# andreaskoepf/CLIP-Image-Captioning

Measured on NVIDIA B200. Metric: captions/sec (GPT2-XL, prefix 40, 32 tok), higher is better.
Workload: dtype bf16

## Files before the change

### clip-image-captioning_b200/csrc/engine.cu

```cuda
#include <stdarg.h>
#include <stdio.h>
#include <stdlib.h>
#include <string.h>

#include <algorithm>

#include "engine.h"

using namespace ccb;

namespace {

thread_local char g_create_err[512] = "";

int fail(ccb_ctx* c, const char* fmt, ...) {
  char buf[512];
  va_list ap;
  va_start(ap, fmt);
  vsnprintf(buf, sizeof(buf), fmt, ap);
  va_end(ap);
  if (c)
    c->err = buf;
  else
    snprintf(g_create_err, sizeof(g_create_err), "%s", buf);
// ... 397 lines not shown
  p.tbl_entries = m.tbl_entries;
  for (int k = 0; k < 4; ++k) p.g[k] = m.g[k];
  p.h = c->h;
  p.x = c->x;
  p.att = c->att;
  p.mlp = c->mlp;
  p.ws = m.d_ws;
  p.wte = c->wte;
  p.wpe = c->wpe;
  p.tokens = c->next_tokens;
  p.ctx_len = c->ctx_len;
  p.block_table = c->block_table;
  p.kv = c->kv;
  p.lnf_g = c->lm_lnf.g;
  p.lnf_b = c->lm_lnf.b;
  p.sync = m.d_sync;
  p.sc_cap = (c->max_pages_per_row + 3) & ~3;
  p.trace = m.trace;
  p.log2_page_tokens = 0;
  while ((1 << p.log2_page_tokens) < c->kv.page_tokens) ++p.log2_page_tokens;
  RUN(mega_launch(p, s));
  return 0;
}

int lm_decode_step(ccb_ctx* c, int rows, cudaStream_t s) {
  const ccb_model_desc& D = c->desc;
  const int d = D.lm_d, H = D.lm_heads, hd = d / H;
  if (c->mega.available && rows <= c->mega.max_rows && c->mega.enabled && (c->kv.page_tokens & (c->kv.page_tokens - 1)) == 0) {
    if (lm_decode_layers_mega(c, rows, s)) return -1;
    RUN(linear(c, c->x, d, rows, c->lm_head, CCB_ACT_NONE, nullptr, 0, c->logits, c->ldv, 0, s));
    return 0;
  }
  RUN(embed_tokens(c->wte, D.lm_arch == CCB_LM_GPT2 ? c->wpe : nullptr, c->next_tokens, c->ctx_len, c->h, rows, d, D.lm_vocab, D.lm_n_pos, s));
  const BlockShape sh = lm_shape(D);
  const float scale = 1.0f / sqrtf(static_cast<float>(hd));
  static const bool fuse_out = [] {
    const char* e = getenv("CCB_GPTJ_FUSE_OUT");
    return !(e && e[0] == '0');
  }();
  for (int l = 0; l < D.lm_layers; ++l) {
    const Block& b = c->lm[l];
    if (sh.parallel && fuse_out && b.projfc2.w != nullptr && c->attmlp != nullptr) {
      const long long ldc = 5LL * d;
      RUN(layernorm_f32_bf16(c->h, d, b.ln1.g, b.ln1.b, sh.eps, c->x, d, rows, d, s));
      RUN(linear(c, c->x, d, rows, b.qkv, CCB_ACT_NONE, nullptr, 0, c->qkv, 3 * d, 1, s));
      RUN(attention_decode(c->qkv, c->attmlp, ldc, rows, H, hd, scale, &c->kv, l, c->block_table, c->ctx_len, D.lm_rotary_dim, s));
      RUN(linear(c, c->x, d, rows, b.fc, sh.act, nullptr, 0, c->attmlp + d, ldc, 1, s));
      RUN(linear(c, c->attmlp, ldc, rows, b.projfc2, CCB_ACT_NONE, c->h, d, c->h, d, 0, s));
      continue;
    }
    auto attn = [&]() {
      return attention_decode(c->qkv, c->att, d, rows, H, hd, scale, &c->kv, l, c->block_table, c->ctx_len,
                              D.lm_rotary_dim, s);
    };
    if (block_forward(c, b, rows, sh, attn, s)) return -1;
  }
  RUN(layernorm_f32_bf16(c->h, d, c->lm_lnf.g, c->lm_lnf.b, D.lm_ln_eps, c->x, d, rows, d, s));
  RUN(linear(c, c->x, d, rows, c->lm_head, CCB_ACT_NONE, nullptr, 0, c->logits, c->ldv, 0, s));
  return 0;
}

SampleParams sample_params(ccb_ctx* c, const ccb_gen_params* p, int rows) {
  SampleParams sp;
  sp.temperature = p->temperature;
  sp.top_p = p->top_p;
  sp.top_k = p->top_k;
  sp.top_p_rows = p->top_p_rows;
  sp.top_k_rows = p->top_k_rows;
  sp.typ_p = p->typ_p;
  sp.typ_p_rows = p->typ_p_rows;
  sp.repetition_penalty = p->repetition_penalty;
  sp.q_noise = p->q_noise;
  sp.ldq = p->q_ld;
  sp.q_step_stride = static_cast<long long>(rows) * p->q_ld;
  sp.seed = p->seed;
  sp.row_ids = reinterpret_cast<const long long*>(p->row_ids);
  (void)c;
  return sp;
}

int select_step(ccb_ctx* c, const ccb_gen_params* p, int rows, int T, bool after_prefill, cudaStream_t s) {
  const int V = c->desc.lm_vocab;
  if (p->mode == CCB_GEN_GREEDY) {
    RUN(sample_greedy(c->logits, c->ldv, rows, V, c->next_tokens, s));
  } else {
    SampleParams sp = sample_params(c, p, rows);
    sp.history = c->gen_tokens;
    sp.ld_hist = T;
    sp.hist_len_from_step = 1;
    sp.step = c->step;
    RUN(sample_top_p(c->logits, c->ldv, rows, V, sp, c->next_tokens, s));
  }
  RUN(advance_rows(c->next_tokens, rows, c->gen_tokens, T, c->lengths, c->stops, c->finished,
                   after_prefill ? nullptr : c->ctx_len, c->step, p->stop_token, p->max_stops, p->eos_token, s));
  return 0;
}

int beam_select(ccb_ctx* c, const ccb_gen_params* p, int N, int T, bool first, cudaStream_t s) {
  const int beam = p->beam_size, rows = N * beam;
  if (!first) RUN(increment_rows(c->ctx_len, rows, c->step, s));
  BeamState st;
  st.scores = c->scores;
  st.seq_lengths = c->seq_lengths;
  st.has_stopped = c->has_stopped;
  st.tokens = c->gen_tokens;
  st.max_len = T;
  st.step = c->step;
  st.cand_scratch = c->beam_cand;
  st.cand_rows = c->max_rows;
  if (c->capturing) c->capture_launches++; else c->launches++;
  RUN(beam_step(c->logits, c->ldv, N, beam, c->desc.lm_vocab, p->temperature, p->stop_token, st, c->next_tokens,
                c->src_rows, c->block_table, c->max_pages_per_row, c->ctx_len, s));
  return 0;
}

int decode_iteration(ccb_ctx* c, const ccb_gen_params* p, int N, int rows, int T, cudaStream_t s) {
  if (lm_decode_step(c, rows, s)) return -1;
  if (p->mode == CCB_GEN_BEAM) return beam_select(c, p, N, T, false, s);
  return select_step(c, p, rows, T, false, s);
}

std::string graph_key(const ccb_gen_params* p, int N, int rows, int T, int c_mega) {
  char buf[512];
  snprintf(buf, sizeof(buf), "g%d m%d N%d r%d T%d st%d ms%d eos%d t%a p%a k%d rp%a b%d seed%llu q%p ld%lld ids%p pr%p kr%p ty%a tr%p",
           c_mega, p->mode, N, rows, T, p->stop_token, p->max_stops, p->eos_token, p->temperature, p->top_p, p->top_k,
           p->repetition_penalty, p->beam_size, static_cast<unsigned long long>(p->seed),
           static_cast<const void*>(p->q_noise), static_cast<long long>(p->q_ld), static_cast<const void*>(p->row_ids),
           static_cast<const void*>(p->top_p_rows), static_cast<const void*>(p->top_k_rows), p->typ_p,
           static_cast<const void*>(p->typ_p_rows));
  return buf;
}

int generate_on_work_stream(ccb_ctx* c, const ccb_gen_params* p, const float* embeds, int N, int S0,
                            int32_t* tokens_out, int32_t* lengths_out, float* scores_out) {
  const ccb_model_desc& D = c->desc;
  cudaStream_t s = c->work;
  const bool is_beam = p->mode == CCB_GEN_BEAM;
  const int beam = is_beam ? p->beam_size : 1;
  const int rows = N * beam;
  const int T = p->max_new_tokens;
  if (p->mode != CCB_GEN_GREEDY && p->mode != CCB_GEN_SAMPLE && !is_beam) return fail(c, "generate: unknown mode %d", p->mode);
  if (N <= 0 || N > D.max_images) return fail(c, "generate: N=%d outside [1, max_images=%d]", N, D.max_images);
  if (beam < 1 || beam > D.max_beam || beam > 8) return fail(c, "generate: beam_size=%d outside [1, max_beam=%d]", beam, D.max_beam);
  if (T <= 0 || S0 <= 0 || S0 + T > D.max_ctx) return fail(c, "generate: S0=%d + max_new_tokens=%d exceeds max_ctx=%d", S0, T, D.max_ctx);
  if (N * S0 > D.max_lm_tokens) return fail(c, "generate: N*S0=%d exceeds max_lm_tokens=%d", N * S0, D.max_lm_tokens);
  if (const char* why = attention_prefill_unsupported(S0, D.lm_d / D.lm_heads, 1, true, D.lm_rotary_dim, false))
    return fail(c, "generate: prefix of S0=%d tokens with head_dim %d: %s", S0, D.lm_d / D.lm_heads, why);

  const int page_tokens = is_beam ? 1 : D.page_tokens;
  const int pages_per_row = is_beam ? (S0 + T) : (S0 + T + page_tokens - 1) / page_tokens;
  const long long need_tokens = is_beam ? static_cast<long long>(N) * (S0 + static_cast<long long>(beam) * T)
                                        : static_cast<long long>(rows) * pages_per_row * page_tokens;
  if (need_tokens > c->kv_pool_tokens) return fail(c, "generate: KV pool too small (%lld > %lld tokens)", need_tokens, c->kv_pool_tokens);
  c->kv.page_tokens = page_tokens;
  c->kv.num_pages = static_cast<int>(c->kv_pool_tokens / page_tokens);
  c->kv.max_pages_per_row = c->max_pages_per_row;

  init_state_kernel<<<148, 256, 0, s>>>(c->block_table, c->block_table_prefill, c->max_pages_per_row, rows, N, beam, S0,
                                        T, page_tokens, pages_per_row, c->ctx_len, c->step, c->lengths, c->stops,
                                        c->finished, c->scores, c->seq_lengths, c->has_stopped);
  RUN(launch_check());
  CUDA_OK(cudaMemsetAsync(c->gen_tokens, 0, sizeof(int) * static_cast<size_t>(rows) * T, s));

  const int slot = static_cast<int>(c->generate_calls % ccb_ctx::kTimingSlots);
  CUDA_OK(cudaEventRecord(c->ev_t0[slot], s));
  if (lm_prefill_layers(c, embeds, N, S0, nullptr, true, s)) return -1;
  if (lm_logits(c, N, S0, 1, c->logits, c->ldv, s)) return -1;
  if (is_beam) {
    if (beam_select(c, p, N, T, true, s)) return -1;
  } else {
    if (select_step(c, p, rows, T, true, s)) return -1;
  }
  CUDA_OK(cudaEventRecord(c->ev_t1[slot], s));

  if (T > 1) {
// ... 301 lines not shown
    make_linear(c, a, c->vit_proj, D.vit_out, w, false);
    add_slot(c, "visual.proj", WeightSlot::MATRIX_T, c->vit_proj.w, w, D.vit_out, w);
  }

  if (D.text_present) {
    const int w = D.text_width;
    c->txt_wte = a.arr<bf16>(static_cast<size_t>(D.text_vocab) * w);
    c->txt_wpe = a.arr<bf16>(static_cast<size_t>(D.text_ctx) * w);
    add_slot(c, "clip_text.token_embedding.weight", WeightSlot::ROWS_BF16, c->txt_wte, D.text_vocab, w, w);
    add_slot(c, "clip_text.positional_embedding", WeightSlot::ROWS_BF16, c->txt_wpe, D.text_ctx, w, w);
    make_ln(a, c->txt_ln_final, w);
    slot_ln(c, "clip_text.ln_final", c->txt_ln_final, w);
    c->txt.resize(D.text_layers);
    for (int l = 0; l < D.text_layers; ++l) {
      Block& b = c->txt[l];
      const std::string base = fmt("clip_text.transformer.resblocks.%d", l);
      make_ln(a, b.ln1, w);
      make_ln(a, b.ln2, w);
      slot_ln(c, base + ".ln_1", b.ln1, w);
      slot_ln(c, base + ".ln_2", b.ln2, w);
      make_linear(c, a, b.qkv, 3 * w, w, true);
      make_linear(c, a, b.proj, w, w, true);
      make_linear(c, a, b.fc, 4 * w, w, true);
      make_linear(c, a, b.fc2, w, 4 * w, true);
      add_slot(c, base + ".attn.in_proj_weight", WeightSlot::MATRIX, b.qkv.w, 3 * w, w, w);
      add_slot(c, base + ".attn.in_proj_bias", WeightSlot::VECTOR_F32, b.qkv.bias, 3 * w, 1, 1);
      slot_linear(c, base + ".attn.out_proj", b.proj);
      slot_linear(c, base + ".mlp.c_fc", b.fc);
      slot_linear(c, base + ".mlp.c_proj", b.fc2);
    }
    make_linear(c, a, c->txt_proj, D.text_out, w, false);
    add_slot(c, "clip_text.text_projection", WeightSlot::MATRIX_T, c->txt_proj.w, w, D.text_out, w);
    c->txt_positions = a.arr<int>(static_cast<size_t>(D.max_texts) * D.text_ctx);
    c->txt_eot = a.arr<int>(D.max_texts);
  }

  c->max_rows = D.max_images * D.max_beam;
  int M = std::max(D.max_lm_tokens, c->max_rows);
  M = std::max(M, D.max_images * map_S);
  M = std::max(M, D.max_images * vit_S);
  if (D.text_present) M = std::max(M, D.max_texts * D.text_ctx);
  c->max_rows_tokens = M;
  c->dmax = std::max(d, std::max(D.vit_present ? D.vit_width : 0, D.text_present ? D.text_width : 0));
  c->hidden_max = std::max(4 * d, std::max(D.map_kind != CCB_MAP_NONE ? (D.map_act == CCB_ACT_GEGLU ? 2 : 1) * D.map_hidden : 0,
                                           D.vit_present ? 4 * D.vit_width : 0));
  if (D.text_present) c->hidden_max = std::max(c->hidden_max, 4 * D.text_width);
  const size_t Mz = static_cast<size_t>(M);
  c->h = a.arr<float>(Mz * c->dmax);
  c->x = a.arr<bf16>(Mz * c->dmax);
  c->qkv = a.arr<bf16>(Mz * 3 * c->dmax);
  c->att = a.arr<bf16>(Mz * c->dmax);
  c->mlp = a.arr<bf16>(Mz * c->hidden_max);
  if (D.lm_arch == CCB_LM_GPTJ) c->attmlp = a.arr<bf16>(static_cast<size_t>(c->max_rows) * 5 * d);
  if (D.vit_present) {
    const int g = D.vit_image / D.vit_patch, np = g * g;
    c->patches = a.arr<bf16>(static_cast<size_t>(D.max_images) * np * vit_patch_k(D.vit_patch));
    c->patch_emb = a.arr<float>(static_cast<size_t>(D.max_images) * np * D.vit_width);
  }
  const int dc = std::max(D.map_dim_clip, D.vit_present ? D.vit_out : 0);
  const int feat_tokens = D.map_kind == CCB_MAP_TRANSFORMER_ALL ? std::max(D.map_clip_len, vit_S) : 1;
  c->feat = a.arr<float>(static_cast<size_t>(D.max_images) * feat_tokens * std::max(dc, 1));
  c->feat_bf16 = a.arr<bf16>(static_cast<size_t>(D.max_images) * feat_tokens * std::max(dc, 1));
  c->prefix = a.arr<float>(static_cast<size_t>(D.max_images) * (std::max(D.map_prefix_len, 0) + 1) * d);
  c->ldv = (static_cast<int64_t>(V) + 63) / 64 * 64;
  c->logits = a.arr<float>(static_cast<size_t>(std::max(c->max_rows, D.max_images)) * c->ldv);
  c->gemm_ws.ws_bytes = static_cast<size_t>(96) << 20;
  c->gemm_ws.ws = static_cast<float*>(a.take(c->gemm_ws.ws_bytes));
  c->gemm_ws.sem_count = 8192;
  c->gemm_ws.sem = a.arr<int>(c->gemm_ws.sem_count);
  c->gemm_ws.num_sms = c->num_sms;

  const int lm_H = D.lm_heads;
  c->kv.L = D.lm_layers;
  c->kv.H = lm_H;
  c->kv.hd = lm_hd;
  const long long ctx_round = (static_cast<long long>(D.max_ctx) + D.page_tokens - 1) / D.page_tokens * D.page_tokens;
  c->kv_pool_tokens = static_cast<long long>(c->max_rows) * ctx_round;
  c->kv.base = a.arr<bf16>(static_cast<size_t>(2) * D.lm_layers * c->kv_pool_tokens * d);
  c->max_pages_per_row = D.max_ctx;
  c->block_table = a.arr<int>(static_cast<size_t>(c->max_rows) * c->max_pages_per_row);
  c->block_table_prefill = a.arr<int>(static_cast<size_t>(D.max_images) * c->max_pages_per_row);
  c->ctx_len = a.arr<int>(c->max_rows);
  c->step = a.arr<int>(1);
  c->next_tokens = a.arr<int>(c->max_rows);
  c->src_rows = a.arr<int>(c->max_rows);
  c->beam_cand = a.take(static_cast<size_t>(c->max_rows) * kBeamCandPerRow * 8);
  c->gen_tokens = a.arr<int>(static_cast<size_t>(c->max_rows) * D.max_ctx);
  c->lengths = a.arr<int>(c->max_rows);
  c->stops = a.arr<int>(c->max_rows);
  c->finished = a.arr<uint8_t>(c->max_rows);
  c->scores = a.arr<float>(c->max_rows);
  c->seq_lengths = a.arr<float>(c->max_rows);
  c->has_stopped = a.arr<uint8_t>(c->max_rows);
  c->bos_token = a.arr<int>(D.max_images);

  MegaState& mg = c->mega;
  if (D.lm_arch == CCB_LM_GPT2 && lm_hd == 64 && d <= 4096 && mega_init() == 0) {
    mega_plan(mg, d, 4 * d, c->num_sms);
    if (mg.tbl_entries <= 256) {
      mg.max_rows = std::min(c->max_rows, 256);
      mg.d_wmaps = static_cast<CUtensorMap*>(a.take(sizeof(CUtensorMap) * 4 * D.lm_layers));
      mg.d_layers = a.arr<MegaLayer>(D.lm_layers);
      mg.d_tbl = a.arr<uint32_t>(mg.tbl_entries);
      mg.d_ws = a.arr<float>(mg.ws_floats_per_row * mg.max_rows);
      mg.d_sync = a.arr<unsigned int>(64);
      mg.available = true;
      mg.enabled = mega_enabled();
    }
  }

  if (!a.ok) {
    fail(nullptr, "ccb_create: out of device memory after %lld bytes", static_cast<long long>(c->device_bytes));
    ccb_destroy(c);
    return -1;
  }
  for (size_t i = 0; i < c->allocs.size(); ++i) cudaMemset(c->allocs[i], 0, c->alloc_sizes[i]);
  if (mg.available) {
    std::vector<CUtensorMap> maps(static_cast<size_t>(4) * D.lm_layers);
    std::vector<MegaLayer> lys(D.lm_layers);
    bool ok = true;
    for (int l = 0; l < D.lm_layers && ok; ++l) {
      const Block& b = c->lm[l];
      const Linear* lin[4] = {&b.qkv, &b.proj, &b.fc, &b.fc2};
      for (int k = 0; k < 4; ++k)
        ok = ok && gemm_make_tmap(&maps[l * 4 + k], lin[k]->w, lin[k]->features, lin[k]->K, lin[k]->K, 128) == 0;
      lys[l] = MegaLayer{b.ln1.g, b.ln1.b, b.ln2.g, b.ln2.b, b.qkv.bias, b.proj.bias, b.fc.bias, b.fc2.bias};
    }
    ok = ok && cudaMemcpy(mg.d_wmaps, maps.data(), maps.size() * sizeof(CUtensorMap), cudaMemcpyHostToDevice) == cudaSuccess;
    ok = ok && cudaMemcpy(mg.d_layers, lys.data(), lys.size() * sizeof(MegaLayer), cudaMemcpyHostToDevice) == cudaSuccess;
    ok = ok && cudaMemcpy(mg.d_tbl, mg.h_tbl.data(), mg.h_tbl.size() * sizeof(uint32_t), cudaMemcpyHostToDevice) == cudaSuccess;
    if (!ok) {
      fail(nullptr, "ccb_create: persistent decode kernel setup failed: %s", gemm_last_error());
      ccb_destroy(c);
      return -1;
    }
  }
  if (cudaStreamCreateWithFlags(&c->work, cudaStreamNonBlocking) != cudaSuccess ||
      cudaEventCreateWithFlags(&c->ev_in, cudaEventDisableTiming) != cudaSuccess ||
      cudaEventCreateWithFlags(&c->ev_out, cudaEventDisableTiming) != cudaSuccess ||
      cudaDeviceSynchronize() != cudaSuccess) {
    fail(nullptr, "ccb_create: stream / event creation failed: %s", cudaGetErrorString(cudaGetLastError()));
    ccb_destroy(c);
    return -1;
  }
  for (int i = 0; i < ccb_ctx::kTimingSlots; ++i) {
    if (cudaEventCreate(&c->ev_t0[i]) != cudaSuccess || cudaEventCreate(&c->ev_t1[i]) != cudaSuccess ||
        cudaEventCreate(&c->ev_t2[i]) != cudaSuccess) {
      fail(nullptr, "ccb_create: event creation failed");
      ccb_destroy(c);
      return -1;
    }
  }
  *out = c;
  return 0;
}

int ccb_load_weight(ccb_ctx* c, const char* name, const void* dev_ptr, int dtype, const int64_t* shape, int ndim,
                    void* stream) {
  if (!c || !name || !dev_ptr || !shape) return fail(c, "ccb_load_weight: null argument");
  DeviceGuard dev_guard(c->device);
  cudaStream_t s = static_cast<cudaStream_t>(stream);
  std::string key;
  const char* rest = nullptr;
  if (starts_with(name, "language_model.", &rest)) key = rest;
  else if (starts_with(name, "visual_encoder.", &rest)) key = std::string("visual.") + rest;
  else key = name;
// ... 316 lines not shown
```

### clip-image-captioning_b200/csrc/engine.h

```cpp
#pragma once
#include <cuda_runtime.h>
#include <stdint.h>

#include <string>
#include <unordered_map>
#include <vector>

#include "../../include/clipcap_b200.h"
#include "internal.h"
#include "mega.h"

namespace ccb {

struct Linear {
  bf16* w = nullptr;
  float* bias = nullptr;
  int features = 0, K = 0;
  bool has_bias = false;
  long long ldw = 0;
};
struct LayerNormW {
  float* g = nullptr;
  float* b = nullptr;
};
// ... 2 lines not shown
  Linear qkv, proj, fc, fc2;
  Linear projfc2;
};

struct WeightSlot {
  enum Kind { MATRIX, MATRIX_T, VECTOR_F32, ROWS_BF16 } kind = MATRIX;
  void* dst = nullptr;
  long long rows = 0;
  long long cols = 0;
  long long dst_ld = 0;
  bool* flag = nullptr;
  bool loaded = false;
  bool optional = false;
};

struct GraphEntry {
  cudaGraphExec_t exec = nullptr;
  int nodes = 0;
};

}

struct ccb_ctx {
  ccb_model_desc desc;
  int device = 0;
  int num_sms = 148;
  std::string err;

  std::vector<void*> allocs;
  std::vector<size_t> alloc_sizes;
  int64_t device_bytes = 0;

  std::unordered_map<std::string, ccb::WeightSlot> slots;
  ccb::bf16* wte = nullptr;
  ccb::bf16* wpe = nullptr;
  std::vector<ccb::Block> lm;
  ccb::LayerNormW lm_lnf;
  ccb::Linear lm_head;
  ccb::Linear map_linear;
  ccb::Linear map_mlp2;
  float* map_pos = nullptr;
  bool map_pos_present = false;
  float* map_prefix_const = nullptr;
  std::vector<ccb::Block> mapper;
  ccb::Linear vit_conv;
  float* vit_cls = nullptr;
  float* vit_pos = nullptr;
  ccb::LayerNormW vit_ln_pre, vit_ln_post;
  std::vector<ccb::Block> vit;
  ccb::Linear vit_proj;
  ccb::bf16* txt_wte = nullptr;
  ccb::bf16* txt_wpe = nullptr;
  std::vector<ccb::Block> txt;
  ccb::LayerNormW txt_ln_final;
  ccb::Linear txt_proj;
  int* txt_positions = nullptr;
  int* txt_eot = nullptr;

  int max_rows_tokens = 0;
  int dmax = 0, hidden_max = 0;
  float* h = nullptr;
  ccb::bf16* x = nullptr;
  ccb::bf16* qkv = nullptr;
  ccb::bf16* att = nullptr;
  ccb::bf16* mlp = nullptr;
  ccb::bf16* attmlp = nullptr;
  ccb::bf16* patches = nullptr;
  float* patch_emb = nullptr;
  float* feat = nullptr;
  ccb::bf16* feat_bf16 = nullptr;
  float* prefix = nullptr;
  float* logits = nullptr;
  int64_t ldv = 0;
  ccb::GemmWorkspace gemm_ws;

  ccb::KvCache kv;
  long long kv_pool_tokens = 0;
  int max_rows = 0;
  int max_pages_per_row = 0;
  int* block_table = nullptr;
  int* block_table_prefill = nullptr;
  int* ctx_len = nullptr;
  int* step = nullptr;
  int* next_tokens = nullptr;
  int* src_rows = nullptr;
  void* beam_cand = nullptr;
  int* gen_tokens = nullptr;
  int* lengths = nullptr;
  int* stops = nullptr;
  uint8_t* finished = nullptr;
  float* scores = nullptr;
  float* seq_lengths = nullptr;
  uint8_t* has_stopped = nullptr;
  int* bos_token = nullptr;

  ccb::MegaState mega;

  cudaStream_t work = nullptr;
  cudaEvent_t ev_in = nullptr, ev_out = nullptr;
  static constexpr int kTimingSlots = 64;
  cudaEvent_t ev_t0[kTimingSlots] = {}, ev_t1[kTimingSlots] = {}, ev_t2[kTimingSlots] = {};
  int timing_steps[kTimingSlots] = {};
  long long generate_calls = 0;
  std::unordered_map<std::string, ccb::GraphEntry> graphs;
  int64_t launches = 0;
  bool capturing = false;
  int capture_launches = 0;
};
```

### clip-image-captioning_b200/csrc/internal.h

```cpp
#pragma once
#include <cuda_bf16.h>
#include <cuda_runtime.h>
#include <stdint.h>

namespace ccb {

typedef __nv_bfloat16 bf16;

constexpr int kMaxDevices = 64;
inline int current_device_slot() {
  int d = 0;
  cudaGetDevice(&d);
  return d >= 0 && d < kMaxDevices ? d : 0;
}

bool pdl_enabled();

template <typename... KArgs, typename... Args>
inline cudaError_t launch_kernel(void (*kernel)(KArgs...), dim3 grid, dim3 block, size_t smem, cudaStream_t s, bool pdl,
                                 Args&&... args) {
  cudaLaunchConfig_t cfg = {};
  cfg.gridDim = grid;
  cfg.blockDim = block;
  cfg.dynamicSmemBytes = smem;
// ... 58 lines not shown
int mapper_fill_pos(const float* pos, float* seq, int B, int clip_len, int P, int d, cudaStream_t s);
int cast_f32_bf16(const float* x, long long ldx, bf16* y, long long ldy, int rows, int d, cudaStream_t s);
int geglu_inplace(bf16* x, long long ldx, int rows, int h, cudaStream_t s);
int embed_tokens(const bf16* wte, const bf16* wpe, const int* tokens, const int* positions, float* h, int rows, int d,
                 int vocab, int n_pos, cudaStream_t s);
int add_positions(const float* src, const bf16* wpe, int pos0, int S, float* h, int rows, int d, cudaStream_t s);
int gather_rows_f32(const float* src, long long lds, int gi, int go, int off, float* dst, long long ldd, int rows,
                    int d, cudaStream_t s);

int convert_rows_bf16(const void* src, int dtype, long long rows, int cols, bf16* dst, long long dst_ld,
                      cudaStream_t s);
int convert_f32(const void* src, int dtype, long long n, float* dst, cudaStream_t s);
int transpose_bf16(const void* src, int dtype, int R, int C, bf16* dst , long long dst_ld, cudaStream_t s);

size_t preprocess_scratch_bytes(int H, int W, int new_h, int new_w, int n_px);
int preprocess_image(const uint8_t* rgb, int H, int W, int new_h, int new_w, int top, int left, int n_px, const float* mean,
                     const float* stdv, float* out, void* scratch, size_t scratch_bytes, cudaStream_t s);

struct KvCache {
  bf16* base = nullptr;
  int L = 0, H = 0, hd = 0, page_tokens = 0, num_pages = 0;
  int max_pages_per_row = 0;
  size_t layer_stride() const { return 2ull * num_pages * H * page_tokens * hd; }
  size_t kv_stride() const { return 1ull * num_pages * H * page_tokens * hd; }
};
int attention_prefill(const bf16* qkv, bf16* out, int B, int S, int H, int hd, float scale, int causal,
                      const KvCache* cache, int layer, const int* block_table, int pos0, int rotary_dim,
                      const uint8_t* key_mask, cudaStream_t s);
const char* attention_prefill_unsupported(int S, int hd, int causal, bool cache, int rotary_dim, bool key_mask);
int attention_prefill_long(const bf16* qkv, bf16* out, int B, int S, int H, int hd, float scale, cudaStream_t s);
int attention_decode(const bf16* qkv, bf16* out, long long ldo, int B, int H, int hd, float scale, const KvCache* cache, int layer,
                     const int* block_table, const int* ctx_len, int rotary_dim, cudaStream_t s);

struct SamplerScratch {
  void* buf = nullptr;
  size_t bytes = 0;
};
int sample_greedy(const float* logits, long long ld, int B, int V, int* next, cudaStream_t s);
int cross_entropy(const float* logits, long long ld, int rows, int V, const int* targets, const int* row_map, int ignore_index,
                  float* row_loss, float* out2, cudaStream_t s);
struct SampleParams {
  float temperature = 1.f;
  float top_p = 0.f;
  int top_k = 0;
  const float* top_p_rows = nullptr;
  const int* top_k_rows = nullptr;
  float typ_p = 0.f;
  const float* typ_p_rows = nullptr;
  float repetition_penalty = 1.f;
  const int* history = nullptr;
  long long ld_hist = 0;
  const int* hist_len = nullptr;
  int hist_len_scalar = 0;
  int hist_len_from_step = 0;
  const float* q_noise = nullptr;
  long long ldq = 0;
  long long q_step_stride = 0;
  unsigned long long seed = 0;
  const long long* row_ids = nullptr;
  const int* step = nullptr;
  int step_scalar = 0;
  float* filtered_out = nullptr;
  int* alt_out = nullptr;
};
int sample_top_p(const float* logits, long long ld, int B, int V, const SampleParams& sp, int* next,
                 cudaStream_t s);
struct BeamState {
  float* scores = nullptr;
  float* seq_lengths = nullptr;
  uint8_t* has_stopped = nullptr;
  int* tokens = nullptr;
  int max_len = 0;
  const int* step = nullptr;
  void* cand_scratch = nullptr;
  int cand_rows = 0;
};
constexpr int kBeamCandPerRow = 8;
int beam_step(const float* logits, long long ld, int N, int beam, int V, float temperature, int stop_token,
              const BeamState& st, int* next_tokens , int* src_rows ,
              int* block_table , int max_pages,
              const int* ctx_len , cudaStream_t s);
int advance_rows(const int* next, int rows, int* tokens_out, int max_len, int* lengths, int* stops, uint8_t* finished,
                 int* ctx_len, int* step, int stop_token, int max_stops, int eos_token, cudaStream_t s);
int increment_rows(int* x, int rows, int* scalar, cudaStream_t s);

}
```

### clip-image-captioning_b200/csrc/sampler.cu

```cuda
#include <float.h>

#include "common.cuh"
#include "internal.h"
#include "ptx.cuh"

namespace ccb {

namespace {

constexpr int kSampThreads = 1024;

__device__ __forceinline__ uint32_t order_key(float x) {
  const uint32_t u = __float_as_uint(x);
  return (u & 0x80000000u) ? ~u : (u | 0x80000000u);
}

__device__ __forceinline__ uint4 philox4x32_10(uint4 ctr, uint2 key) {
  const uint32_t M0 = 0xD2511F53u, M1 = 0xCD9E8D57u, W0 = 0x9E3779B9u, W1 = 0xBB67AE85u;
#pragma unroll
  for (int r = 0; r < 10; ++r) {
    const uint32_t hi0 = __umulhi(M0, ctr.x), lo0 = M0 * ctr.x;
    const uint32_t hi1 = __umulhi(M1, ctr.z), lo1 = M1 * ctr.z;
    ctr = make_uint4(hi1 ^ ctr.y ^ key.x, lo1, hi0 ^ ctr.w ^ key.y, lo0);
    key.x += W0;
    key.y += W1;
  }
  return ctr;
}
__device__ __forceinline__ float4 philox_exp1_x4(unsigned long long seed, unsigned long long row, uint32_t step, uint32_t g) {
  const uint4 c = make_uint4(g, step, static_cast<uint32_t>(row), static_cast<uint32_t>(row >> 32));
  const uint2 k = make_uint2(static_cast<uint32_t>(seed), static_cast<uint32_t>(seed >> 32));
  const uint4 r = philox4x32_10(c, k);
  const float sc = 1.0f / 16777216.0f;
  return make_float4(-logf((static_cast<float>(r.x >> 8) + 0.5f) * sc), -logf((static_cast<float>(r.y >> 8) + 0.5f) * sc),
                     -logf((static_cast<float>(r.z >> 8) + 0.5f) * sc), -logf((static_cast<float>(r.w >> 8) + 0.5f) * sc));
}
__device__ __forceinline__ float philox_exp1(unsigned long long seed, unsigned long long row, uint32_t step,
                                             uint32_t v) {
  const uint4 c = make_uint4(v >> 2, step, static_cast<uint32_t>(row), static_cast<uint32_t>(row >> 32));
  const uint2 k = make_uint2(static_cast<uint32_t>(seed), static_cast<uint32_t>(seed >> 32));
  const uint4 r = philox4x32_10(c, k);
  const uint32_t w = (v & 3) == 0 ? r.x : (v & 3) == 1 ? r.y : (v & 3) == 2 ? r.z : r.w;
  const float u = (static_cast<float>(w >> 8) + 0.5f) * (1.0f / 16777216.0f);
  return -logf(u);
}

struct ArgMax {
  float v;
  int i;
};
__device__ __forceinline__ ArgMax argmax_better(ArgMax a, ArgMax b) {
  if (b.v > a.v || (b.v == a.v && b.i < a.i)) return b;
  return a;
}
__device__ __forceinline__ ArgMax block_argmax(ArgMax a, ArgMax* scratch ) {
  const int lane = threadIdx.x & 31, w = threadIdx.x >> 5, nw = (blockDim.x + 31) >> 5;
#pragma unroll
  for (int o = 16; o > 0; o >>= 1) {
    ArgMax b;
    b.v = __shfl_xor_sync(0xffffffffu, a.v, o);
    b.i = __shfl_xor_sync(0xffffffffu, a.i, o);
    a = argmax_better(a, b);
  }
  __syncthreads();
  if (lane == 0) scratch[w] = a;
  __syncthreads();
  ArgMax r;
  r.v = -INFINITY;
  r.i = 0x7fffffff;
  if (lane < nw) r = scratch[lane];
#pragma unroll
  for (int o = 16; o > 0; o >>= 1) {
    ArgMax b;
    b.v = __shfl_xor_sync(0xffffffffu, r.v, o);
    b.i = __shfl_xor_sync(0xffffffffu, r.i, o);
    r = argmax_better(r, b);
  }
  return r;
}

__device__ __forceinline__ double warp_sum_d(double v) {
#pragma unroll
  for (int o = 16; o > 0; o >>= 1) v += __shfl_xor_sync(0xffffffffu, v, o);
  return v;
}
__device__ __forceinline__ double block_sum_d(double v, double* scratch ) {
  const int lane = threadIdx.x & 31, w = threadIdx.x >> 5, nw = (blockDim.x + 31) >> 5;
  v = warp_sum_d(v);
  __syncthreads();
  if (lane == 0) scratch[w] = v;
  __syncthreads();
  double r = (lane < nw) ? scratch[lane] : 0.0;
  return warp_sum_d(r);
}
__device__ __forceinline__ int block_sum_i(int v, int* scratch) {
  const int lane = threadIdx.x & 31, w = threadIdx.x >> 5, nw = (blockDim.x + 31) >> 5;
#pragma unroll
  for (int o = 16; o > 0; o >>= 1) v += __shfl_xor_sync(0xffffffffu, v, o);
  __syncthreads();
  if (lane == 0) scratch[w] = v;
  __syncthreads();
  int r = (lane < nw) ? scratch[lane] : 0;
#pragma unroll
  for (int o = 16; o > 0; o >>= 1) r += __shfl_xor_sync(0xffffffffu, r, o);
  return r;
}

__global__ void __launch_bounds__(kSampThreads) greedy_kernel(const float* __restrict__ logits, long long ld, int V,
                                                              int* __restrict__ next) {
  __shared__ ArgMax scratch[32];
  ptx::grid_dep_wait();
  ptx::grid_dep_launch();
  const float* row = logits + static_cast<long long>(blockIdx.x) * ld;
  ArgMax a;
  a.v = -INFINITY;
  a.i = 0x7fffffff;
  int v_done = 0;
  if ((reinterpret_cast<uintptr_t>(row) & 15) == 0) {
    const float4* row4 = reinterpret_cast<const float4*>(row);
    const int nq = V >> 2;
    for (int q0 = threadIdx.x; q0 < nq; q0 += 4 * kSampThreads) {
      float4 w[4];
#pragma unroll
      for (int j = 0; j < 4; ++j) {
        const int q = q0 + j * kSampThreads;
        w[j] = q < nq ? row4[q] : make_float4(-INFINITY, -INFINITY, -INFINITY, -INFINITY);
      }
#pragma unroll
      for (int j = 0; j < 4; ++j) {
        const int q = q0 + j * kSampThreads;
        if (q >= nq) continue;
        const float e[4] = {w[j].x, w[j].y, w[j].z, w[j].w};
#pragma unroll
        for (int k = 0; k < 4; ++k) {
          ArgMax b;
          b.v = e[k];
          b.i = 4 * q + k;
          a = argmax_better(a, b);
        }
      }
    }
    v_done = nq << 2;
  }
  for (int v = v_done + threadIdx.x; v < V; v += blockDim.x) {
    ArgMax b;
    b.v = row[v];
    b.i = v;
    a = argmax_better(a, b);
  }
  a = block_argmax(a, scratch);
  if (threadIdx.x == 0) next[blockIdx.x] = a.i;
}

__global__ void __launch_bounds__(kSampThreads) cross_entropy_rows_kernel(const float* __restrict__ logits, long long ld, int V,
                                                                          const int* __restrict__ targets, const int* __restrict__ row_map,
                                                                          int ignore_index, float* __restrict__ row_loss) {
  __shared__ ArgMax ascratch[32];
  __shared__ double dscratch[32];
  const int r = blockIdx.x;
  const int tgt = targets[r];
  if (tgt == ignore_index || tgt < 0 || tgt >= V) {
    if (threadIdx.x == 0) row_loss[r] = 0.f;
    return;
  }
  const float* row = logits + static_cast<long long>(row_map ? row_map[r] : r) * ld;
  ArgMax a;
  a.v = -INFINITY;
  a.i = 0x7fffffff;
  for (int v = threadIdx.x; v < V; v += kSampThreads) {
    ArgMax b;
    b.v = row[v];
    b.i = v;
    a = argmax_better(a, b);
  }
  a = block_argmax(a, ascratch);
  const float vmax = a.v;
  double sum = 0.0;
  for (int v = threadIdx.x; v < V; v += kSampThreads) sum += static_cast<double>(expf(row[v] - vmax));
  sum = block_sum_d(sum, dscratch);
  if (threadIdx.x == 0) row_loss[r] = static_cast<float>(static_cast<double>(vmax) + log(sum) - static_cast<double>(row[tgt]));
}

__global__ void __launch_bounds__(kSampThreads) cross_entropy_mean_kernel(const float* __restrict__ row_loss, const int* __restrict__ targets,
                                                                          int rows, int ignore_index, float* __restrict__ out) {
  __shared__ double dscratch[32];
  __shared__ int iscratch[32];
  double s = 0.0;
  int n = 0;
  for (int r = threadIdx.x; r < rows; r += kSampThreads) {
    if (targets[r] != ignore_index) {
      s += static_cast<double>(row_loss[r]);
      ++n;
    }
  }
  s = block_sum_d(s, dscratch);
  n = block_sum_i(n, iscratch);
  if (threadIdx.x == 0) {
    out[0] = static_cast<float>(s / static_cast<double>(n));
    out[1] = static_cast<float>(n);
  }
}

struct SelectResult {
  uint32_t key;
  double mass_gt;
  int cnt_eq;
  int reached;
};

__device__ __forceinline__ uint32_t typical_key(float x, float vmax, float lse, float ent) {
  return order_key(-fabsf(((x - vmax) - lse) + ent));
}

__device__ SelectResult radix_select(const float* vals, int V, int mode, int kth, float top_p, float vmax,
                                     float inv_sum, double* dscratch , int* iscratch ,
                                     float lse = 0.f, float ent = 0.f) {
  uint32_t prefix = 0;
  double mass_above = 0.0;
  int cnt_above = 0;
  int reached = 1;
  int cnt_eq = 0;
  double* bin_mass = dscratch + 32;
  int* bin_cnt = iscratch + 32;
  for (int nib = 7; nib >= 0; --nib) {
    const int shift = nib * 4;
    double m[16];
    int c[16];
#pragma unroll
    for (int b = 0; b < 16; ++b) {
      m[b] = 0.0;
      c[b] = 0;
    }
    for (int v = threadIdx.x; v < V; v += blockDim.x) {
      const float x = vals[v];
// ... 702 lines not shown
  if (threadIdx.x < beam) {
    const uint8_t st = first ? 0 : a.has_stopped[n * beam + threadIdx.x];
    s_stop[threadIdx.x] = st;
    s_len[threadIdx.x] = first ? 1.f : a.seq_lengths[n * beam + threadIdx.x] + (st ? 0.f : 1.f);
  }
  if (threadIdx.x == 0) {
    const Cand* cand = a.cand + static_cast<long long>(n) * beam * kMaxBeam;
    int heads[kMaxBeam];
    for (int q = 0; q < kMaxBeam; ++q) heads[q] = 0;
    for (int k = 0; k < beam; ++k) {
      int bw = -1;
      Cand best;
      best.v = -INFINITY;
      best.idx = 0x7fffffff;
      for (int q = 0; q < rows; ++q) {
        if (heads[q] >= beam) continue;
        const Cand c = cand[q * kMaxBeam + heads[q]];
        if (bw < 0 || cand_better(c, best)) {
          best = c;
          bw = q;
        }
      }
      heads[bw]++;
      top[k] = best;
    }
  }
  __syncthreads();

  __shared__ int s_src[kMaxBeam], s_tok[kMaxBeam];
  if (threadIdx.x < beam) {
    const int k = threadIdx.x;
    const Cand c = top[k];
    int src, tok;
    float new_len, new_score;
    uint8_t stopped;
    if (first) {
      src = 0;
      tok = c.idx;
      new_len = 1.f;
      new_score = c.v;
      stopped = 0;
    } else {
      src = c.idx / V;
      tok = c.idx % V;
      new_len = s_len[src];
      new_score = c.v * new_len;
      stopped = s_stop[src];
    }
    stopped = stopped | (tok == a.stop_token ? 1 : 0);
    s_src[k] = src;
    s_tok[k] = tok;
    a.scores[n * beam + k] = new_score;
    a.seq_lengths[n * beam + k] = new_len;
    a.has_stopped[n * beam + k] = stopped;
    a.next_tokens[n * beam + k] = tok;
    a.src_rows[n * beam + k] = n * beam + src;
  }
  __syncthreads();
  {
    int* tk = a.tokens + static_cast<long long>(n) * beam * a.max_len;
    if (!first) {
      for (int idx = threadIdx.x; idx < beam * step; idx += blockDim.x) perm_buf[idx] = tk[(idx / step) * a.max_len + idx % step];
      __syncthreads();
      for (int idx = threadIdx.x; idx < beam * step; idx += blockDim.x) {
        const int k = idx / step, t = idx % step;
        tk[k * a.max_len + t] = perm_buf[s_src[k] * step + t];
      }
    }
    if (threadIdx.x < beam && step < a.max_len) tk[threadIdx.x * a.max_len + step] = s_tok[threadIdx.x];
  }
  if (!first && a.block_table != nullptr) {
    __syncthreads();
    const int ctx = a.ctx_len[n * beam];
    int* bt = a.block_table + static_cast<long long>(n) * beam * a.max_pages;
    for (int idx = threadIdx.x; idx < beam * ctx; idx += blockDim.x) perm_buf[idx] = bt[(idx / ctx) * a.max_pages + idx % ctx];
    __syncthreads();
    for (int idx = threadIdx.x; idx < beam * ctx; idx += blockDim.x) {
      const int k = idx / ctx, t = idx % ctx;
      bt[k * a.max_pages + t] = perm_buf[s_src[k] * ctx + t];
    }
  }
}

__global__ void advance_kernel(const int* __restrict__ next, int rows, int* tokens_out, int max_len, int* lengths,
                               int* stops, uint8_t* finished, int* ctx_len, int* step, int stop_token, int max_stops,
                               int eos_token) {
  ptx::grid_dep_wait();
  ptx::grid_dep_launch();
  const int st = *step;
  for (int r = threadIdx.x; r < rows; r += blockDim.x) {
    const int tok = next[r];
    if (tokens_out && st < max_len) tokens_out[static_cast<long long>(r) * max_len + st] = tok;
    if (finished && !finished[r]) {
      int sc = stops[r];
      if (tok == stop_token) sc += 1;
      stops[r] = sc;
      const bool fin = (max_stops > 0 && sc >= max_stops) || (eos_token >= 0 && tok == eos_token);
      lengths[r] = st + 1;
      if (fin) finished[r] = 1;
    }
    if (ctx_len) ctx_len[r] += 1;
  }
  __syncthreads();
  if (threadIdx.x == 0) *step = st + 1;
}

}

int sample_greedy(const float* logits, long long ld, int B, int V, int* next, cudaStream_t s) {
  if (B <= 0) return 0;
  cudaError_t e = launch_kernel(greedy_kernel, dim3(B), dim3(kSampThreads), 0, s, true, logits, ld, V, next);
  return e == cudaSuccess ? 0 : (int)e;
}

int cross_entropy(const float* logits, long long ld, int rows, int V, const int* targets, const int* row_map, int ignore_index,
                  float* row_loss, float* out2, cudaStream_t s) {
  if (rows <= 0) return 0;
  cross_entropy_rows_kernel<<<rows, kSampThreads, 0, s>>>(logits, ld, V, targets, row_map, ignore_index, row_loss);
  cross_entropy_mean_kernel<<<1, kSampThreads, 0, s>>>(row_loss, targets, rows, ignore_index, out2);
  cudaError_t e = cudaGetLastError();
  return e == cudaSuccess ? 0 : (int)e;
}

int sample_top_p(const float* logits, long long ld, int B, int V, const SampleParams& sp, int* next,
                 cudaStream_t s) {
  if (B <= 0) return 0;
  const size_t smem = static_cast<size_t>(V) * sizeof(float);
  if (smem > 208 * 1024) return (int)cudaErrorInvalidValue;
  static bool configured_dev[kMaxDevices] = {};
  bool& configured = configured_dev[current_device_slot()];
  if (!configured) {
    cudaError_t e = cudaFuncSetAttribute(top_p_kernel, cudaFuncAttributeMaxDynamicSharedMemorySize, 208 * 1024);
    if (e != cudaSuccess) return (int)e;
    configured = true;
  }
  TopPArgs a;
  a.logits = logits; a.ld = ld; a.V = V;
  a.temperature = sp.temperature; a.top_p = sp.top_p; a.top_k = sp.top_k;
  a.top_p_rows = sp.top_p_rows; a.top_k_rows = sp.top_k_rows;
  a.typ_p = sp.typ_p; a.typ_p_rows = sp.typ_p_rows;
  a.rep_pen = sp.repetition_penalty; a.history = sp.history; a.ld_hist = sp.ld_hist;
  a.hist_len = sp.hist_len; a.hist_len_scalar = sp.hist_len_scalar; a.hist_len_from_step = sp.hist_len_from_step;
  a.q_noise = sp.q_noise; a.ldq = sp.ldq; a.q_step_stride = sp.q_step_stride; a.seed = sp.seed; a.row_ids = sp.row_ids;
  a.step = sp.step; a.step_scalar = sp.step_scalar;
  a.filtered_out = sp.filtered_out; a.alt_out = sp.alt_out; a.next = next;
  static const bool fast_on = [] {
    const char* e = getenv("CCB_SAMPLER_FAST");
    return !(e && e[0] == '0');
  }();
  a.fast = fast_on ? 1 : 0;
  top_p_kernel<<<B, kSampThreads, smem, s>>>(a);
  cudaError_t e = cudaGetLastError();
  return e == cudaSuccess ? 0 : (int)e;
}

int beam_step(const float* logits, long long ld, int N, int beam, int V, float temperature, int stop_token,
              const BeamState& st, int* next_tokens, int* src_rows, int* block_table, int max_pages,
              const int* ctx_len, cudaStream_t s) {
  if (N <= 0) return 0;
  if (beam < 1 || beam > kMaxBeam) return (int)cudaErrorInvalidValue;
  BeamArgs a;
  a.logits = logits; a.ld = ld; a.beam = beam; a.V = V; a.temperature = temperature; a.stop_token = stop_token;
  a.scores = st.scores; a.seq_lengths = st.seq_lengths; a.has_stopped = st.has_stopped; a.tokens = st.tokens;
  a.max_len = st.max_len; a.step = st.step; a.next_tokens = next_tokens; a.src_rows = src_rows;
  a.block_table = block_table; a.max_pages = max_pages; a.ctx_len = ctx_len;
  if (st.cand_scratch == nullptr || st.cand_rows < N * beam) return (int)cudaErrorInvalidValue;
  a.cand = static_cast<Cand*>(st.cand_scratch);
  const int m = st.max_len > max_pages ? st.max_len : max_pages;
  const size_t smem = static_cast<size_t>(beam) * m * sizeof(int);
  if (smem > 64 * 1024) return (int)cudaErrorInvalidValue;
  static bool configured_dev[kMaxDevices] = {};
  bool& configured = configured_dev[current_device_slot()];
  if (!configured) {
    cudaError_t e = cudaFuncSetAttribute(beam_merge_kernel, cudaFuncAttributeMaxDynamicSharedMemorySize, 64 * 1024);
    if (e != cudaSuccess) return (int)e;
    configured = true;
  }
  beam_rows_kernel<<<N * beam, kBeamRowThreads, 0, s>>>(a);
  beam_merge_kernel<<<N, 256, smem, s>>>(a);
  cudaError_t e = cudaGetLastError();
  return e == cudaSuccess ? 0 : (int)e;
}

__global__ void increment_kernel(int* x, int rows, int* scalar) {
  for (int r = threadIdx.x; r < rows; r += blockDim.x) x[r] += 1;
  if (scalar && threadIdx.x == 0) *scalar += 1;
}
}
namespace ccb {
int increment_rows(int* x, int rows, int* scalar, cudaStream_t s) {
  increment_kernel<<<1, 1024, 0, s>>>(x, rows, scalar);
  cudaError_t e = cudaGetLastError();
  return e == cudaSuccess ? 0 : (int)e;
}

int advance_rows(const int* next, int rows, int* tokens_out, int max_len, int* lengths, int* stops, uint8_t* finished,
                 int* ctx_len, int* step, int stop_token, int max_stops, int eos_token, cudaStream_t s) {
  cudaError_t e = launch_kernel(advance_kernel, dim3(1), dim3(1024), 0, s, true, next, rows, tokens_out, max_len, lengths,
                                stops, finished, ctx_len, step, stop_token, max_stops, eos_token);
  return e == cudaSuccess ? 0 : (int)e;
}

}
```

Measured before the change: 766.0.

## Fuse greedy argmax with row advance using last-block atomic counter

Greedy decoding now runs one kernel per step that computes each row's argmax and immediately updates that row's token history, stop counters and context length, instead of launching a separate single-block advance kernel. A global atomic counter finds the last finishing block, which bumps the step counter and resets the counter. The argmax loop also keeps 8 float4 loads in flight instead of 4. This removes one kernel launch and its dependency latency per decode step, at the cost of an atomic, thread fences and the assumption that the counter starts at zero.

```diff
diff --git a/clip-image-captioning_b200/csrc/engine.cu b/clip-image-captioning_b200/csrc/engine.cu
--- a/clip-image-captioning_b200/csrc/engine.cu
+++ b/clip-image-captioning_b200/csrc/engine.cu
@@ -503,15 +503,17 @@
 int select_step(ccb_ctx* c, const ccb_gen_params* p, int rows, int T, bool after_prefill, cudaStream_t s) {
   const int V = c->desc.lm_vocab;
   if (p->mode == CCB_GEN_GREEDY) {
-    RUN(sample_greedy(c->logits, c->ldv, rows, V, c->next_tokens, s));
-  } else {
-    SampleParams sp = sample_params(c, p, rows);
-    sp.history = c->gen_tokens;
-    sp.ld_hist = T;
-    sp.hist_len_from_step = 1;
-    sp.step = c->step;
-    RUN(sample_top_p(c->logits, c->ldv, rows, V, sp, c->next_tokens, s));
-  }
+    RUN(greedy_advance_rows(c->logits, c->ldv, V, c->next_tokens, rows, c->gen_tokens, T, c->lengths, c->stops, c->finished,
+                            after_prefill ? nullptr : c->ctx_len, c->step, c->rows_done, p->stop_token, p->max_stops,
+                            p->eos_token, s));
+    return 0;
+  }
+  SampleParams sp = sample_params(c, p, rows);
+  sp.history = c->gen_tokens;
+  sp.ld_hist = T;
+  sp.hist_len_from_step = 1;
+  sp.step = c->step;
+  RUN(sample_top_p(c->logits, c->ldv, rows, V, sp, c->next_tokens, s));
   RUN(advance_rows(c->next_tokens, rows, c->gen_tokens, T, c->lengths, c->stops, c->finished,
                    after_prefill ? nullptr : c->ctx_len, c->step, p->stop_token, p->max_stops, p->eos_token, s));
   return 0;
@@ -979,6 +981,7 @@
   c->block_table_prefill = a.arr<int>(static_cast<size_t>(D.max_images) * c->max_pages_per_row);
   c->ctx_len = a.arr<int>(c->max_rows);
   c->step = a.arr<int>(1);
+  c->rows_done = a.arr<int>(1);
   c->next_tokens = a.arr<int>(c->max_rows);
   c->src_rows = a.arr<int>(c->max_rows);
   c->beam_cand = a.take(static_cast<size_t>(c->max_rows) * kBeamCandPerRow * 8);
diff --git a/clip-image-captioning_b200/csrc/engine.h b/clip-image-captioning_b200/csrc/engine.h
--- a/clip-image-captioning_b200/csrc/engine.h
+++ b/clip-image-captioning_b200/csrc/engine.h
@@ -108,6 +108,7 @@
   int* block_table_prefill = nullptr;
   int* ctx_len = nullptr;
   int* step = nullptr;
+  int* rows_done = nullptr;
   int* next_tokens = nullptr;
   int* src_rows = nullptr;
   void* beam_cand = nullptr;
diff --git a/clip-image-captioning_b200/csrc/internal.h b/clip-image-captioning_b200/csrc/internal.h
--- a/clip-image-captioning_b200/csrc/internal.h
+++ b/clip-image-captioning_b200/csrc/internal.h
@@ -164,6 +164,9 @@
               const int* ctx_len , cudaStream_t s);
 int advance_rows(const int* next, int rows, int* tokens_out, int max_len, int* lengths, int* stops, uint8_t* finished,
                  int* ctx_len, int* step, int stop_token, int max_stops, int eos_token, cudaStream_t s);
+int greedy_advance_rows(const float* logits, long long ld, int V, int* next, int rows, int* tokens_out, int max_len,
+                        int* lengths, int* stops, uint8_t* finished, int* ctx_len, int* step, int* rows_done, int stop_token,
+                        int max_stops, int eos_token, cudaStream_t s);
 int increment_rows(int* x, int rows, int* scalar, cudaStream_t s);
 
 }
diff --git a/clip-image-captioning_b200/csrc/sampler.cu b/clip-image-captioning_b200/csrc/sampler.cu
--- a/clip-image-captioning_b200/csrc/sampler.cu
+++ b/clip-image-captioning_b200/csrc/sampler.cu
@@ -106,12 +106,33 @@
   return r;
 }
 
-__global__ void __launch_bounds__(kSampThreads) greedy_kernel(const float* __restrict__ logits, long long ld, int V,
-                                                              int* __restrict__ next) {
-  __shared__ ArgMax scratch[32];
-  ptx::grid_dep_wait();
-  ptx::grid_dep_launch();
-  const float* row = logits + static_cast<long long>(blockIdx.x) * ld;
+struct AdvanceArgs {
+  int rows;
+  int* tokens_out;
+  int max_len;
+  int *lengths, *stops;
+  uint8_t* finished;
+  int* ctx_len;
+  int* step;
+  int* rows_done;
+  int stop_token, max_stops, eos_token;
+};
+
+__device__ __forceinline__ void advance_row(const AdvanceArgs& g, int r, int st, int tok) {
+  if (g.tokens_out && st < g.max_len) g.tokens_out[static_cast<long long>(r) * g.max_len + st] = tok;
+  if (g.finished && !g.finished[r]) {
+    int sc = g.stops[r];
+    if (tok == g.stop_token) sc += 1;
+    g.stops[r] = sc;
+    const bool fin = (g.max_stops > 0 && sc >= g.max_stops) || (g.eos_token >= 0 && tok == g.eos_token);
+    g.lengths[r] = st + 1;
+    if (fin) g.finished[r] = 1;
+  }
+  if (g.ctx_len) g.ctx_len[r] += 1;
+}
+
+__device__ __forceinline__ ArgMax row_argmax(const float* row, int V, ArgMax* scratch) {
+  constexpr int kInFlight = 8;
   ArgMax a;
   a.v = -INFINITY;
   a.i = 0x7fffffff;
@@ -119,15 +140,15 @@
   if ((reinterpret_cast<uintptr_t>(row) & 15) == 0) {
     const float4* row4 = reinterpret_cast<const float4*>(row);
     const int nq = V >> 2;
-    for (int q0 = threadIdx.x; q0 < nq; q0 += 4 * kSampThreads) {
-      float4 w[4];
-#pragma unroll
-      for (int j = 0; j < 4; ++j) {
+    for (int q0 = threadIdx.x; q0 < nq; q0 += kInFlight * kSampThreads) {
+      float4 w[kInFlight];
+#pragma unroll
+      for (int j = 0; j < kInFlight; ++j) {
         const int q = q0 + j * kSampThreads;
         w[j] = q < nq ? row4[q] : make_float4(-INFINITY, -INFINITY, -INFINITY, -INFINITY);
       }
 #pragma unroll
-      for (int j = 0; j < 4; ++j) {
+      for (int j = 0; j < kInFlight; ++j) {
         const int q = q0 + j * kSampThreads;
         if (q >= nq) continue;
         const float e[4] = {w[j].x, w[j].y, w[j].z, w[j].w};
@@ -148,8 +169,37 @@
     b.i = v;
     a = argmax_better(a, b);
   }
-  a = block_argmax(a, scratch);
+  return block_argmax(a, scratch);
+}
+
+__global__ void __launch_bounds__(kSampThreads) greedy_kernel(const float* __restrict__ logits, long long ld, int V,
+                                                              int* __restrict__ next) {
+  __shared__ ArgMax scratch[32];
+  ptx::grid_dep_wait();
+  ptx::grid_dep_launch();
+  const ArgMax a = row_argmax(logits + static_cast<long long>(blockIdx.x) * ld, V, scratch);
   if (threadIdx.x == 0) next[blockIdx.x] = a.i;
+}
+
+__global__ void __launch_bounds__(kSampThreads) greedy_advance_kernel(const float* __restrict__ logits, long long ld, int V,
+                                                                      int* __restrict__ next, AdvanceArgs g) {
+  __shared__ ArgMax scratch[32];
+  ptx::grid_dep_wait();
+  ptx::grid_dep_launch();
+  const int r = blockIdx.x;
+  const ArgMax a = row_argmax(logits + static_cast<long long>(r) * ld, V, scratch);
+  if (threadIdx.x == 0) {
+    const int st = *g.step;
+    const int tok = a.i;
+    next[r] = tok;
+    advance_row(g, r, st, tok);
+    __threadfence();
+    if (atomicAdd(g.rows_done, 1) == g.rows - 1) {
+      __threadfence();
+      *g.step = st + 1;
+      *g.rows_done = 0;
+    }
+  }
 }
 
 __global__ void __launch_bounds__(kSampThreads) cross_entropy_rows_kernel(const float* __restrict__ logits, long long ld, int V,
@@ -1018,27 +1068,13 @@
   }
 }
 
-__global__ void advance_kernel(const int* __restrict__ next, int rows, int* tokens_out, int max_len, int* lengths,
-                               int* stops, uint8_t* finished, int* ctx_len, int* step, int stop_token, int max_stops,
-                               int eos_token) {
+__global__ void advance_kernel(const int* __restrict__ next, AdvanceArgs g) {
   ptx::grid_dep_wait();
   ptx::grid_dep_launch();
-  const int st = *step;
-  for (int r = threadIdx.x; r < rows; r += blockDim.x) {
-    const int tok = next[r];
-    if (tokens_out && st < max_len) tokens_out[static_cast<long long>(r) * max_len + st] = tok;
-    if (finished && !finished[r]) {
-      int sc = stops[r];
-      if (tok == stop_token) sc += 1;
-      stops[r] = sc;
-      const bool fin = (max_stops > 0 && sc >= max_stops) || (eos_token >= 0 && tok == eos_token);
-      lengths[r] = st + 1;
-      if (fin) finished[r] = 1;
-    }
-    if (ctx_len) ctx_len[r] += 1;
-  }
-  __syncthreads();
-  if (threadIdx.x == 0) *step = st + 1;
+  const int st = *g.step;
+  for (int r = threadIdx.x; r < g.rows; r += blockDim.x) advance_row(g, r, st, next[r]);
+  __syncthreads();
+  if (threadIdx.x == 0) *g.step = st + 1;
 }
 
 }
@@ -1130,11 +1166,43 @@
   return e == cudaSuccess ? 0 : (int)e;
 }
 
+namespace {
+AdvanceArgs advance_args(int rows, int* tokens_out, int max_len, int* lengths, int* stops, uint8_t* finished, int* ctx_len,
+                         int* step, int* rows_done, int stop_token, int max_stops, int eos_token) {
+  AdvanceArgs g;
+  g.rows = rows;
+  g.tokens_out = tokens_out;
+  g.max_len = max_len;
+  g.lengths = lengths;
+  g.stops = stops;
+  g.finished = finished;
+  g.ctx_len = ctx_len;
+  g.step = step;
+  g.rows_done = rows_done;
+  g.stop_token = stop_token;
+  g.max_stops = max_stops;
+  g.eos_token = eos_token;
+  return g;
+}
+}
+
 int advance_rows(const int* next, int rows, int* tokens_out, int max_len, int* lengths, int* stops, uint8_t* finished,
                  int* ctx_len, int* step, int stop_token, int max_stops, int eos_token, cudaStream_t s) {
-  cudaError_t e = launch_kernel(advance_kernel, dim3(1), dim3(1024), 0, s, true, next, rows, tokens_out, max_len, lengths,
-                                stops, finished, ctx_len, step, stop_token, max_stops, eos_token);
+  const AdvanceArgs g = advance_args(rows, tokens_out, max_len, lengths, stops, finished, ctx_len, step, nullptr, stop_token,
+                                     max_stops, eos_token);
+  cudaError_t e = launch_kernel(advance_kernel, dim3(1), dim3(1024), 0, s, true, next, g);
   return e == cudaSuccess ? 0 : (int)e;
 }
 
-}
+int greedy_advance_rows(const float* logits, long long ld, int V, int* next, int rows, int* tokens_out, int max_len,
+                        int* lengths, int* stops, uint8_t* finished, int* ctx_len, int* step, int* rows_done, int stop_token,
+                        int max_stops, int eos_token, cudaStream_t s) {
+  if (rows <= 0) return 0;
+  if (rows_done == nullptr) return (int)cudaErrorInvalidValue;
+  const AdvanceArgs g = advance_args(rows, tokens_out, max_len, lengths, stops, finished, ctx_len, step, rows_done, stop_token,
+                                     max_stops, eos_token);
+  cudaError_t e = launch_kernel(greedy_advance_kernel, dim3(rows), dim3(kSampThreads), 0, s, true, logits, ld, V, next, g);
+  return e == cudaSuccess ? 0 : (int)e;
+}
+
+}
```

New measurement: 766.8, median of 6. No clear change (+0.1%).
